# cvxgrp/pymde

Hardware: AMD Instinct MI355X
Metric: edges/sec/iter (avg_distortion fwd+bwd), n=1M |E|=50M d=2 (higher is better)
Workload: dtype f32; 1 GPU; BASELINE configs[3] / SURVEY 8d config 4a: n=1000000, |E|=50000000 uniform-random edges (out-degree 50), d=2, penalties.Log1p(1.5), weights in {1,2}; seeded on the device with torch.Generator(0) (the survey's recipe uses numpy default_rng(0): same distribution, another stream; --survey-seed builds that one); parallelism=single GPU, parameter_stream=codebook: 2 distinct weights ride in the packed half-edge word (4 B/half-edge)

## Files before the change

### include/mde_hip.h

```cpp
#ifndef MDE_HIP_H_
#define MDE_HIP_H_

#include <stdint.h>

#ifdef __cplusplus
extern "C" {
#endif

#define MDE_ABI_VERSION 2

#define MDE_OK 0
#define MDE_E_INVALID (-1)
#define MDE_E_SELF_EDGE (-2)
#define MDE_E_RANGE (-3)
#define MDE_E_TOO_LARGE (-4)
#define MDE_E_HIP (-5)
#define MDE_E_UNSUPPORTED (-6)

const char* mde_last_error(void);
int mde_abi_version(void);

enum {
  MDE_F_NONE = 0,
  MDE_F_LINEAR = 1,
// ... 21 lines not shown
  MDE_F_L_LOGISTIC = 39,
  MDE_F_L_FRACTIONAL = 40,
  MDE_F_L_SOFT_FRACTIONAL = 41,
  MDE_F_L_CLIPPED_QUADRATIC = 42,
  MDE_F_L_LOG1P = 43
};

typedef struct mde_func {
  int32_t kind;
  int32_t kind_neg;
  const float* a0;
  const float* a1;
  int32_t a0_scalar;
  int32_t a1_scalar;
  float s0, s1, s2;
  float n0, n1, n2;
  int32_t layout;
  const float* e0;
  const float* e1;
} mde_func;

typedef struct mde_plan mde_plan;

int mde_plan_create(int64_t n, int64_t p, const int64_t* edges, int64_t row_lo, int64_t row_hi,
                    void* stream, mde_plan** out);
int mde_plan_destroy(mde_plan* plan);
int64_t mde_plan_n(const mde_plan* plan);
int64_t mde_plan_p(const mde_plan* plan);
int64_t mde_plan_half_edges(const mde_plan* plan);
int64_t mde_plan_row_lo(const mde_plan* plan);
int64_t mde_plan_row_hi(const mde_plan* plan);
const int32_t* mde_plan_rowptr(const mde_plan* plan);
const int32_t* mde_plan_nbr(const mde_plan* plan);
const int32_t* mde_plan_eid(const mde_plan* plan);

int mde_plan_export(const mde_plan* plan, int32_t* rowptr_out, int32_t* nbr_out, int32_t* eid_out,
                    void* stream);

int mde_shard_bounds(int64_t n, int64_t p, const int64_t* edges, int32_t world,
                     int64_t* bounds_host, void* stream);

int mde_plan_expand(const mde_plan* plan, const float* in_edge, float* out_half, void* stream);

int mde_plan_layout(mde_plan* plan, int32_t d, void* stream);
int mde_plan_function_hint(mde_plan* plan, int32_t kind, int32_t kind_neg);
int64_t mde_plan_layout_half_edges(const mde_plan* plan, int32_t layout);
int mde_plan_expand_codebook(const mde_plan* plan, const float* in_edge, float* out_half,
                             int32_t* n_values_host, void* stream);
int mde_plan_expand_bytes(const mde_plan* plan, const float* in_edge, float* out_half,
                          int32_t* n_values_host, void* stream);
int mde_plan_expand_layout(const mde_plan* plan, int32_t layout, const float* in_edge,
                           float* out_half, void* stream);
int mde_plan_ring_info(const mde_plan* plan, int64_t* info_host);
int mde_plan_row_order(mde_plan* plan, int32_t mode, void* stream, double* info_host);
int mde_plan_loss_double(const mde_plan* plan, double* dst, void* stream);

int mde_edges_deduplicate(int64_t n, int64_t p, const int64_t* edges, int64_t* edges_out,
                          int64_t* count_host, void* stream);
int mde_edges_count_unique(int64_t n, int64_t p, const int64_t* edges, int64_t* edges_out,
                           float* weights_out, int64_t* count_host, void* stream);
int mde_knn(int64_t n, int32_t nf, const float* data, int32_t k, int32_t* idx_out, float* d2_out,
            float* sqn_work, void* stream);
int mde_row_sqnorm(int64_t n, int32_t nf, const float* data, float* out, void* stream);
int mde_ann_search(int32_t nf, int32_t k, int32_t flags, int64_t n_q, const float* Q, const float* q_sqn,
                   int64_t n_qpos, const int32_t* q_map, int64_t n_b, const float* B, const float* b_sqn,
                   int64_t n_bpos, const int32_t* b_map, int64_t n_lists, const int64_t* offsets,
                   int32_t n_probe, const int32_t* probe, int64_t n_tiles, const int64_t* tiles,
                   int32_t* idx_out, float* d2_out, void* stream);
int mde_ann_centroids(int64_t n, int32_t nf, const float* data, int64_t n_members, const int32_t* members,
                      int64_t n_lists, const int64_t* offsets, float* centroids, void* stream);
int mde_sparse_validate(int64_t n, int32_t nf, int64_t nnz, const int64_t* indptr, const int32_t* indices,
                        const float* values, void* stream);
int mde_sparse_knn(int64_t n, int32_t nf, int64_t nnz, const int64_t* indptr, const int32_t* indices,
                   const float* values, int32_t k, int32_t* idx_out, float* d2_out, float* sqn_work,
                   void* stream);
int mde_sparse_distances(int64_t n, int32_t nf, int64_t nnz, const int64_t* indptr, const int32_t* indices,
                         const float* values, int64_t p, const int64_t* edges, float* out, void* stream);
int mde_graph_shortest_paths(const mde_plan* plan, const float* w, float max_length,
                             double retain_fraction, uint64_t seed, int64_t capacity,
                             int64_t* edges_out, float* dist_out, int64_t* count_host, void* stream);
int mde_knn_pairs(int64_t n, int32_t k, const int32_t* idx, const float* val, float max_value,
                  int64_t* pairs_out, void* stream);
int mde_graph_knn(const mde_plan* plan, const float* w, float max_length, int32_t direct, int32_t k,
                  int32_t* idx_out, float* dist_out, void* stream);
int mde_sample_edges(int64_t n, int64_t num_edges, uint64_t seed, const int64_t* exclude,
                     int64_t n_exclude, int64_t* edges_out, int64_t* count_host, void* stream);

int mde_average_distortion(mde_plan* plan, const float* X, int32_t d, const mde_func* f,
                           float grad_scale, float* grad, float* loss_out, void* stream);

int mde_differences(int64_t n, int64_t p, const int64_t* edges, const float* X, int32_t d,
                    float* diff_out , void* stream);
int mde_distances(int64_t n, int64_t p, const int64_t* edges, const float* X, int32_t d,
                  float* dist_out , void* stream);
int mde_distances_backward(const mde_plan* plan, const float* X, int32_t d, const float* gout,
                           float* grad , void* stream);
int mde_distortions(int64_t p, const float* dist, const mde_func* f, float* out, float* dout,
                    void* stream);

int mde_scatter(const mde_plan* plan, const float* X, int32_t d, const float* gnorm,
                const float* dist, float scale, float* grad, void* stream);

int mde_center(int64_t n, int32_t d, float* Z, double* work, void* stream);
int mde_anchor_rows(int64_t n_anchors, int32_t d, const int64_t* anchors, const float* values,
                    float* Z, void* stream);
int mde_sphere_rows(int64_t n, int32_t d, const float* X, float* Z, float radius, void* stream);
// ... 83 lines not shown
```

### pymde_amd/_lib.py

```python
import ctypes
import os
import threading

import torch

_HERE = os.path.dirname(os.path.abspath(__file__))
LIB_PATH = os.path.join(_HERE, "libmde_hip.so")

c_i32, c_i64, c_f32 = ctypes.c_int32, ctypes.c_int64, ctypes.c_float
c_vp = ctypes.c_void_p

MDE_OK = 0
MDE_E_INVALID, MDE_E_SELF_EDGE, MDE_E_RANGE = -1, -2, -3
MDE_E_TOO_LARGE, MDE_E_HIP, MDE_E_UNSUPPORTED = -4, -5, -6


class MdeFunc(ctypes.Structure):
    _fields_ = [("kind", c_i32), ("kind_neg", c_i32), ("a0", c_vp), ("a1", c_vp),
                ("a0_scalar", c_i32), ("a1_scalar", c_i32),
                ("s0", c_f32), ("s1", c_f32), ("s2", c_f32),
                ("n0", c_f32), ("n1", c_f32), ("n2", c_f32), ("layout", c_i32),
                ("e0", c_vp), ("e1", c_vp)]


class MdeTurnDesc(ctypes.Structure):
    _fields_ = [("plan", c_vp), ("func", c_vp), ("n", c_i64), ("d", c_i32), ("kind", c_i32),
                ("X", c_vp * 2), ("g", c_vp), ("g_prev", c_vp), ("dir", c_vp), ("loss_dev", c_vp),
                ("board", c_vp), ("work", c_vp), ("status", c_vp), ("lbfgs", c_vp),
                ("host_dst", c_vp), ("tail_src", c_vp), ("read_bytes", c_i64),
                ("host_loss", c_vp), ("host_status", c_vp), ("host_board", c_vp), ("seq", ctypes.c_double),
                ("pre_id", ctypes.c_double)]


SYMBOLS = {
    "mde_last_error": (ctypes.c_char_p, []),
    "mde_abi_version": (c_i32, []),
    "mde_plan_create": (c_i32, [c_i64, c_i64, c_vp, c_i64, c_i64, c_vp, ctypes.POINTER(c_vp)]),
    "mde_plan_destroy": (c_i32, [c_vp]),
    "mde_plan_n": (c_i64, [c_vp]),
    "mde_plan_p": (c_i64, [c_vp]),
    "mde_plan_half_edges": (c_i64, [c_vp]),
    "mde_plan_row_lo": (c_i64, [c_vp]),
    "mde_plan_row_hi": (c_i64, [c_vp]),
    "mde_plan_rowptr": (c_vp, [c_vp]),
    "mde_plan_nbr": (c_vp, [c_vp]),
    "mde_plan_eid": (c_vp, [c_vp]),
    "mde_plan_export": (c_i32, [c_vp, c_vp, c_vp, c_vp, c_vp]),
    "mde_shard_bounds": (c_i32, [c_i64, c_i64, c_vp, c_i32, ctypes.POINTER(c_i64), c_vp]),
    "mde_plan_expand": (c_i32, [c_vp, c_vp, c_vp, c_vp]),
    "mde_plan_layout": (c_i32, [c_vp, c_i32, c_vp]),
    "mde_plan_layout_half_edges": (c_i64, [c_vp, c_i32]),
    "mde_plan_ring_info": (c_i32, [c_vp, ctypes.POINTER(c_i64)]),
    "mde_plan_row_order": (c_i32, [c_vp, c_i32, c_vp, ctypes.POINTER(ctypes.c_double)]),
    "mde_plan_function_hint": (c_i32, [c_vp, c_i32, c_i32]),
    "mde_plan_loss_double": (c_i32, [c_vp, c_vp, c_vp]),
    "mde_center_step_begin": (c_i32, [c_i64, c_i32, c_vp, c_vp, c_f32, c_vp, c_vp, c_vp]),
    "mde_center_step_end": (c_i32, [c_i64, c_i32, c_vp, c_vp, ctypes.c_double, c_vp]),
    "mde_lbfgs_dev_stage": (c_i32, [c_vp, c_vp, c_vp, c_vp, c_f32, c_vp, c_vp]),
    "mde_lbfgs_dev_finish": (c_i32, [c_vp, c_vp, c_vp, c_vp, c_vp, c_vp]),
    "mde_lbfgs_dev_dots": (c_i32, [c_vp]),
    "mde_rank_reduce": (c_i32, [c_i32, c_i32, ctypes.c_uint64, c_vp, c_vp, c_i32, c_vp, c_vp]),
    "mde_plan_expand_codebook": (c_i32, [c_vp, c_vp, c_vp, ctypes.POINTER(c_i32), c_vp]),
    "mde_plan_expand_bytes": (c_i32, [c_vp, c_vp, c_vp, ctypes.POINTER(c_i32), c_vp]),
    "mde_plan_expand_layout": (c_i32, [c_vp, c_i32, c_vp, c_vp, c_vp]),
    "mde_edges_deduplicate": (c_i32, [c_i64, c_i64, c_vp, c_vp, ctypes.POINTER(c_i64), c_vp]),
    "mde_edges_count_unique": (c_i32, [c_i64, c_i64, c_vp, c_vp, c_vp, ctypes.POINTER(c_i64), c_vp]),
    "mde_knn": (c_i32, [c_i64, c_i32, c_vp, c_i32, c_vp, c_vp, c_vp, c_vp]),
    "mde_row_sqnorm": (c_i32, [c_i64, c_i32, c_vp, c_vp, c_vp]),
    "mde_ann_search": (c_i32, [c_i32, c_i32, c_i32, c_i64, c_vp, c_vp, c_i64, c_vp, c_i64, c_vp, c_vp, c_i64, c_vp,
                               c_i64, c_vp, c_i32, c_vp, c_i64, c_vp, c_vp, c_vp, c_vp]),
    "mde_ann_centroids": (c_i32, [c_i64, c_i32, c_vp, c_i64, c_vp, c_i64, c_vp, c_vp, c_vp]),
    "mde_knn_pairs": (c_i32, [c_i64, c_i32, c_vp, c_vp, c_f32, c_vp, c_vp]),
    "mde_sparse_validate": (c_i32, [c_i64, c_i32, c_i64, c_vp, c_vp, c_vp, c_vp]),
    "mde_sparse_knn": (c_i32, [c_i64, c_i32, c_i64, c_vp, c_vp, c_vp, c_i32, c_vp, c_vp, c_vp, c_vp]),
    "mde_sparse_distances": (c_i32, [c_i64, c_i32, c_i64, c_vp, c_vp, c_vp, c_i64, c_vp, c_vp, c_vp]),
    "mde_graph_knn": (c_i32, [c_vp, c_vp, c_f32, c_i32, c_i32, c_vp, c_vp, c_vp]),
    "mde_graph_shortest_paths": (c_i32, [c_vp, c_vp, c_f32, ctypes.c_double, ctypes.c_uint64, c_i64,
                                         c_vp, c_vp, ctypes.POINTER(c_i64), c_vp]),
    "mde_sample_edges": (c_i32, [c_i64, c_i64, ctypes.c_uint64, c_vp, c_i64, c_vp,
                                 ctypes.POINTER(c_i64), c_vp]),
    "mde_average_distortion": (c_i32, [c_vp, c_vp, c_i32, ctypes.POINTER(MdeFunc), c_f32, c_vp,
                                       c_vp, c_vp]),
    "mde_differences": (c_i32, [c_i64, c_i64, c_vp, c_vp, c_i32, c_vp, c_vp]),
    "mde_distances": (c_i32, [c_i64, c_i64, c_vp, c_vp, c_i32, c_vp, c_vp]),
    "mde_distances_backward": (c_i32, [c_vp, c_vp, c_i32, c_vp, c_vp, c_vp]),
    "mde_distortions": (c_i32, [c_i64, c_vp, ctypes.POINTER(MdeFunc), c_vp, c_vp, c_vp]),
    "mde_scatter": (c_i32, [c_vp, c_vp, c_i32, c_vp, c_vp, c_f32, c_vp, c_vp]),
    "mde_center": (c_i32, [c_i64, c_i32, c_vp, c_vp, c_vp]),
    "mde_anchor_rows": (c_i32, [c_i64, c_i32, c_vp, c_vp, c_vp, c_vp]),
    "mde_sphere_rows": (c_i32, [c_i64, c_i32, c_vp, c_vp, c_f32, c_vp]),
    "mde_std_tangent": (c_i32, [c_i64, c_i32, c_vp, c_vp, c_vp, c_vp]),
    "mde_std_retract": (c_i32, [c_i64, c_i32, c_vp, c_i32, c_vp, c_vp, c_vp]),
    "mde_center_step": (c_i32, [c_i64, c_i32, c_vp, c_vp, c_f32, c_vp, c_vp, c_vp]),
    "mde_std_retract_step": (c_i32, [c_i64, c_i32, c_vp, c_vp, c_f32, c_vp, c_i32, c_vp, c_vp, c_vp]),
    "mde_std_tangent_stats": (c_i32, [c_i64, c_i32, c_vp, c_vp, c_vp, c_vp, c_vp, c_vp]),
    "mde_gram": (c_i32, [c_i64, c_i32, c_i32, c_vp, c_vp, c_vp, c_vp, c_vp]),
    "mde_right_multiply": (c_i32, [c_i64, c_i32, c_i32, c_vp, c_vp, c_vp, c_vp]),
    "mde_right_multiply_add": (c_i32, [c_i64, c_i32, c_i32, c_vp, c_vp, c_f32, c_vp, c_vp, c_vp]),
    "mde_shift_rows": (c_i32, [c_i64, c_i32, c_vp, c_vp, c_vp]),
    "mde_row_scale": (c_i32, [c_i64, c_i32, c_vp, c_vp, c_vp]),
    "mde_weighted_degree": (c_i32, [c_vp, c_vp, c_vp, c_vp]),
    "mde_work_doubles": (c_i64, [c_i32]),
    "mde_axpy": (c_i32, [c_i64, c_f32, c_vp, c_vp, c_vp, c_vp]),
    "mde_vec_stats": (c_i32, [c_i64, c_vp, c_vp, c_vp, c_vp, c_vp, c_vp]),
    "mde_lbfgs_create": (c_i32, [c_i64, c_i32, ctypes.POINTER(c_vp)]),
# ... 79 lines not shown
```

### pymde_amd/average_distortion.py

```python
import ctypes

import torch

from pymde_amd import _lib
from pymde_amd import util


def _check_X(X, n=None, d=None):
    if not isinstance(X, torch.Tensor) or X.dim() != 2:
        raise ValueError("the embedding must be a 2-D tensor")
    if X.dtype != torch.float32:
        raise ValueError(
            "pymde_amd computes in float32; got an embedding of dtype %s (MDE.embed and "
            "MDE.average_distortion cast float64 inputs with a warning; the kernels themselves do not)" % X.dtype)
    util.require_cuda_device(X.device)
    if n is not None and X.shape[0] != n:
        raise ValueError("embedding has %d rows, the problem has %d items" % (X.shape[0], n))


class EdgePlan(object):

    def __init__(self, n_items, edges, row_lo=0, row_hi=None):
        lib = _lib.load()
        device = util.require_cuda_device(edges.device)
# ... 27 lines not shown
    @property
    def is_full(self):
        return self.row_lo == 0 and self.row_hi == self.n

    def expand(self, per_edge, layout=0):
        lib = _lib.load()
        t = per_edge.detach().to(device=self.device, dtype=torch.float32).contiguous().reshape(-1)
        if t.numel() != self.p:
            raise ValueError(
                "distortion function has %d parameters but the problem has %d edges"
                % (t.numel(), self.p))
        size = int(lib.mde_plan_layout_half_edges(self._handle, int(layout)))
        out = torch.empty(max(size, 1), dtype=torch.float32, device=self.device)
        with torch.cuda.device(self.device):
            _lib.check(lib.mde_plan_expand_layout(self._handle, int(layout), _lib.ptr(t),
                                                  _lib.ptr(out), _lib.stream_ptr(self.device)))
        return out

    def expand_codebook(self, per_edge):
        lib = _lib.load()
        t = per_edge.detach().to(device=self.device, dtype=torch.float32).contiguous().reshape(-1)
        if t.numel() != self.p:
            return None
        size = int(lib.mde_plan_layout_half_edges(self._handle, 1))
        out = torch.empty(max(size, 1), dtype=torch.float32, device=self.device)
        nv = ctypes.c_int32(0)
        with torch.cuda.device(self.device):
            _lib.check(lib.mde_plan_expand_codebook(self._handle, _lib.ptr(t), _lib.ptr(out),
                                                    ctypes.byref(nv), _lib.stream_ptr(self.device)))
        return out if nv.value > 0 else None

    def expand_bytes(self, per_edge):
        lib = _lib.load()
        t = per_edge.detach().to(device=self.device, dtype=torch.float32).contiguous().reshape(-1)
        if t.numel() != self.p:
            return None
        size = int(lib.mde_plan_layout_half_edges(self._handle, 1))
        out = torch.empty(max(size, 1), dtype=torch.float32, device=self.device)
        nv = ctypes.c_int32(0)
        with torch.cuda.device(self.device):
            _lib.check(lib.mde_plan_expand_bytes(self._handle, _lib.ptr(t), _lib.ptr(out),
                                                 ctypes.byref(nv), _lib.stream_ptr(self.device)))
        return out if nv.value > 0 else None

    def ring_info(self):
        lib = _lib.load()
        info = (ctypes.c_int64 * 16)()
        _lib.check(lib.mde_plan_ring_info(self._handle, info))
        names = ("built", "d", "rows_per_block", "row_blocks", "col_groups", "chunks", "ring_slots", "iterations",
                 "ring_half_edges", "padded_entries", "permuted", "hub_rows", "hub_half_edges", "hub_segments")
        out = {k: int(info[i]) for i, k in enumerate(names)}
        out["built"], out["permuted"] = bool(out["built"]), bool(out["permuted"])
        return out

    def row_order(self, mode=1):
        lib = _lib.load()
        info = (ctypes.c_double * 4)()
        with torch.cuda.device(self.device):
            _lib.check(lib.mde_plan_row_order(self._handle, int(mode), _lib.stream_ptr(self.device), info))
        return {"in_use": bool(info[0]), "mean_distance_before": float(info[1]),
                "mean_distance_after": float(info[2]), "levels": int(info[3])}

    def csr(self):
        lib = _lib.load()
        nloc = self.row_hi - self.row_lo
        rowptr = torch.empty(nloc + 1, dtype=torch.int32, device=self.device)
        nbr = torch.empty(max(self.half_edges, 1), dtype=torch.int32, device=self.device)
        eid = torch.empty(max(self.half_edges, 1), dtype=torch.int32, device=self.device)
        with torch.cuda.device(self.device):
            _lib.check(lib.mde_plan_export(self._handle, _lib.ptr(rowptr), _lib.ptr(nbr),
                                           _lib.ptr(eid), _lib.stream_ptr(self.device)))
        return rowptr, nbr[:self.half_edges], eid[:self.half_edges]

    def __del__(self):
        h = getattr(self, "_handle", None)
        if h is not None and h.value:
            try:
                _lib.load().mde_plan_destroy(h)
            except Exception:
                pass
            self._handle = None


class Binding(object):

    def __init__(self, plan, function):
        self.plan = plan
        self.function = function
        self.spec = function._hip_spec() if hasattr(function, "_hip_spec") else None
        self._struct = None
        self._keep = None
        self._key = None
        self.codebook = False
        self.byte_stream = False
        self.stream_kind = None

    @property
    def fused(self):
        return self.spec is not None

    def _param_key(self, spec):
        return tuple((a.data_ptr(), a._version, a.numel(), str(a.device)) for a in spec.arrays()) + (
            spec.kind, spec.kind_neg, spec.scalars, spec.scalars_neg)

    def struct(self, d):
        lib = _lib.load()
# ... 186 lines not shown
```

### pymde_amd/csrc/mde_ring.hip

```cpp
#include <algorithm>
#include <chrono>
#include <cmath>
#include <cstring>
#include <vector>

#include "mde_ring.h"

#ifndef MDE_RING_BUCKETS
#define MDE_RING_BUCKETS 32
#endif
__global__ __launch_bounds__(64) void k_ring_assign(int nloc, int R, int Q, int NC, int C, int contiguous,
                                                    const int32_t* __restrict__ rowptr,
                                                    const int32_t* __restrict__ nbr, uint32_t* __restrict__ wmap,
                                                    int32_t* __restrict__ wrows) {
  constexpr int B = MDE_RING_BUCKETS, NCWP = MDE_RING_NCW <= 8 ? 8 : 16, LPW = 64 / NCWP, BPL = B / LPW;
  static_assert(MDE_RING_NCW <= 16 && B % LPW == 0 && B <= 64, "lane map of k_ring_assign");
  __shared__ int hist[B];
  __shared__ float cpre[B];
  const int wg = blockIdx.x, rb = wg / Q, g = wg % Q, lane = threadIdx.x;
  const int j_lo = (int)(((int64_t)g * NC + Q - 1) / Q), j_hi = (int)(((int64_t)(g + 1) * NC + Q - 1) / Q);
  const int nj = max(1, j_hi - j_lo);
  const int r0 = rb * R, nr = min(R, nloc - r0);
  const int w = lane / LPW, bg = lane % LPW;
  uint32_t* out = wmap + (size_t)wg * R;
// ... 343 lines not shown
    caps[i] = 0;
    return;
  }
  const int nrows_w = max(1, wrows[i]);
  const int per_it = nrows_w < 64 ? nrows_w : 64;
  const int walk = 2 * ((NC / Q + SPAN + 1) / (SPAN + 1));
  const int need = max((seg[i + 1] - seg[i] + per_it - 1) / per_it, walk);
  caps[i] = (factor * need + 64 + 4 + 3) & ~3;
}

__device__ __forceinline__ int ring_place_wave(bool act, int rc, int lane) {
  const unsigned long long lt = (1ull << lane) - 1ull;
  int rank = 0, par = 0, oddacc = 0;
  for (int c = 0; c < 32; ++c) {
    const unsigned long long m = __ballot(act && rc == c);
    if (rc == c) {
      rank = __popcll(m & lt);
      par = oddacc & 1;
    }
    oddacc += __popcll(m) & 1;
  }
  const int half = (rank + par) & 1;
  int quarter = 0;
  for (int h = 0; h < 2; ++h) {
    int oa = 0;
    for (int c = 0; c < 16; ++c) {
      const unsigned long long m = __ballot(act && half == h && (rc & 15) == c);
      if (half == h && (rc & 15) == c) quarter = (__popcll(m & lt) + (oa & 1)) & 1;
      oa += __popcll(m) & 1;
    }
  }
  int pos = 0;
  for (int g = 0; g < 4; ++g) {
    const unsigned long long m = __ballot(act && half * 2 + quarter == g);
    if (half * 2 + quarter == g) pos = __popcll(m & lt);
  }
  return half * 32 + quarter * 16 + pos;
}

__global__ __launch_bounds__(MDE_BLOCK) void k_ring_pack(int64_t nit, int nseg, const int32_t* __restrict__ iter_base,
                                                         const int32_t* __restrict__ src_base,
                                                         const int32_t* __restrict__ it_ent,
                                                         const int32_t* __restrict__ it_cnt,
                                                         const int32_t* __restrict__ it_m,
                                                         const uint32_t* __restrict__ keys,
                                                         const uint32_t* __restrict__ vals,
                                                         const int32_t* __restrict__ hrow,
                                                         const int32_t* __restrict__ nbr,
                                                         const int32_t* __restrict__ eid, int R, int Q, int C, int S,
                                                         int ring_off, int JB, int d, int row_lo, int place, int count_all,
                                                         uint32_t* __restrict__ packed,
                                                         int32_t* __restrict__ peid, uint32_t* __restrict__ hdr) {
  __shared__ uint8_t s_taken[MDE_BLOCK / 64][64], s_free[MDE_BLOCK / 64][64];
  const int lane = threadIdx.x & 63, wv = threadIdx.x >> 6;
  const int64_t nw = ((int64_t)gridDim.x * MDE_BLOCK) >> 6;
  const uint32_t JM = (1u << JB) - 1u;
  const int sh = ring_cls_shift(d), cm = ring_cls_mask(d);
  const uint32_t cbytes = (uint32_t)C * 4u * (uint32_t)d;
  for (int64_t itb = (int64_t)blockIdx.x * (MDE_BLOCK / 64); itb < nit; itb += nw) {
    const int64_t it = itb + wv;
    const bool valid = it < nit;
    int64_t src = it;
    if (valid && src_base) {
      int lo = 0, hi = nseg;
      while (hi - lo > 1) {
        const int mid = (lo + hi) >> 1;
        if ((int64_t)iter_base[mid] <= it) lo = mid; else hi = mid;
      }
      src = (int64_t)src_base[lo] + (it - (int64_t)iter_base[lo]);
    }
    const int cw = valid ? __builtin_amdgcn_readfirstlane(it_cnt[src]) : 0;
    const int cnt = cw & 0xff;
    const bool act = valid && lane < cnt;
    uint32_t key = 0, q = 0, col = 0, rowaddr = 0, ring = 0;
    int grow = 0, rcls = 0;
    if (act) {
      const int pos = it_ent[(size_t)src * 64 + lane];
      key = keys[pos];
      q = vals[pos];
      const int rb = (int)((key >> JB) / MDE_RING_NCW) / Q;
      grow = hrow[q];
      rowaddr = (uint32_t)(grow - rb * R) * 4u * (uint32_t)d;
      const uint32_t j = key & JM;
      col = (uint32_t)nbr[q];
      ring = (uint32_t)ring_off + (j % (uint32_t)S) * cbytes + (col - j * (uint32_t)C) * 4u * (uint32_t)d;
      rcls = (int)((rowaddr >> sh) & (uint32_t)cm);
    }
    s_taken[wv][lane] = 0;
    __syncthreads();
    int l = lane;
    if (place) l = ring_place_wave(act, rcls, lane);
    if (act) s_taken[wv][l] = 1;
    __syncthreads();
    {
      const bool fr = !s_taken[wv][lane];
      const unsigned long long fm = __ballot(fr);
      if (fr) s_free[wv][__popcll(fm & ((1ull << lane) - 1ull))] = (uint8_t)lane;
    }
    __syncthreads();
    const bool counts = act && (count_all || (uint32_t)(row_lo + grow) < col);
    const int ncount = __popcll(__ballot(counts));
    const uint32_t lclass = ncount == 0 ? 0u : (ncount == cnt ? 1u : 2u);
    const uint32_t m = valid ? (uint32_t)__builtin_amdgcn_readfirstlane(it_m[src]) : 0u;
    const uint32_t need = max((uint32_t)(cw >> 8), m);
    const uint32_t mpad = valid ? (uint32_t)__builtin_amdgcn_readfirstlane(it_m[src & ~(int64_t)1]) : 0u;
    const size_t base = ((size_t)(it >> 2) * 64) * 4 + (size_t)(it & 3);
    if (act) {
      packed[base + (size_t)l * 4] = ring_pack_word(d, rowaddr, ring);
      peid[base + (size_t)l * 4] = eid[q];
    } else if (valid) {
      const int lf = s_free[wv][lane - cnt];
      packed[base + (size_t)lf * 4] = ring_pack_word(d, (uint32_t)(R + (lf & 31)) * 4u * (uint32_t)d,
                                                     (uint32_t)ring_off + (mpad % (uint32_t)S) * cbytes);
      peid[base + (size_t)lf * 4] = -1;
    }
    if (lane == 0 && valid) {
      hdr[MDE_RING_HW * it] = m;
      hdr[MDE_RING_HW * it + 1] = need;
      hdr[MDE_RING_HW * it + 2] = lclass;
      hdr[MDE_RING_HW * it + 3] = (cnt < 64 ? MDE_RING_H3_PAD : 0u) | ((uint32_t)cnt << 8);
    }
    __syncthreads();
  }
}

__global__ __launch_bounds__(MDE_BLOCK) void k_ring_block_class(int64_t nblocks, uint32_t* __restrict__ hdr) {
  const int64_t b = (int64_t)blockIdx.x * MDE_BLOCK + threadIdx.x;
  if (b >= nblocks) return;
  bool any0 = false, any1 = false, any2 = false;
  for (int q = 0; q < 4; ++q) {
    const uint32_t* h = hdr + (size_t)MDE_RING_HW * (4 * b + q);
    if ((h[3] >> 8) == 0u) continue;
    any0 |= h[2] == 0u;
    any1 |= h[2] == 1u;
    any2 |= h[2] == 2u;
  }
  const uint32_t cls = (any2 || (any0 && any1)) ? 2u : (any1 ? 1u : 0u);
  hdr[(size_t)MDE_RING_HW * 4 * b + 3] = (hdr[(size_t)MDE_RING_HW * 4 * b + 3] & ~3u) | cls;
  for (int t = 0; t < 2; ++t) {
    uint32_t* h0 = hdr + (size_t)MDE_RING_HW * (4 * b + 2 * t);
    uint32_t* h1 = h0 + MDE_RING_HW;
    uint32_t need = h0[0];
    if ((h0[3] >> 8) != 0u) need = max(need, h0[1]);
    if ((h1[3] >> 8) != 0u) need = max(need, h1[1]);
    h0[1] = need;
  }
}

__global__ __launch_bounds__(MDE_BLOCK) void k_ring_stats(int64_t nit, const uint32_t* __restrict__ hdr,
                                                          unsigned long long* __restrict__ stats) {
  unsigned long long a = 0, b = 0, c = 0;
  for (int64_t i = (int64_t)blockIdx.x * MDE_BLOCK + threadIdx.x; i < nit; i += (int64_t)gridDim.x * MDE_BLOCK) {
    a += (hdr[MDE_RING_HW * i + 3] & MDE_RING_H3_PAD) ? 1u : 0u;
    b += hdr[MDE_RING_HW * i + 2] == 1u;
    c += hdr[MDE_RING_HW * i + 2] == 2u;
  }
  a = mde_wave_sum(a);
  b = mde_wave_sum(b);
  c = mde_wave_sum(c);
  if ((threadIdx.x & 63) == 0) {
    atomicAdd(&stats[0], a);
    atomicAdd(&stats[1], b);
    atomicAdd(&stats[2], c);
  }
// ... 982 lines not shown
    memcpy(&fv, &vals[i], sizeof(float));
    if (!std::isfinite(fv) || std::fabs(fv) > 1.0e6f) ok = false;
  }
  if (!ok) {
    (void)hipFree(dtable);
    return MDE_OK;
  }
  std::sort(vals.begin(), vals.end());
  const int nv = (int)vals.size();
  std::vector<unsigned int> tb(MDE_RING_BX_VALUES, 0u);
  for (int i = 0; i < nv; ++i) tb[1 + i] = vals[i];
  unsigned int* table = reinterpret_cast<unsigned int*>(out_half) + L.H / 4;
  err = hipMemcpyAsync(table, tb.data(), MDE_RING_BX_VALUES * sizeof(unsigned int), hipMemcpyHostToDevice, st);
  if (err == hipSuccess) {
    hipLaunchKernelGGL(k_bytes_pack, dim3(mde_grid(L.H, MDE_BLOCK, 4096)), dim3(MDE_BLOCK), 0, st, L.H, L.eid, in_edge, table, nv,
                       reinterpret_cast<uint8_t*>(out_half));
    err = hipGetLastError();
  }
  if (err == hipSuccess) err = hipStreamSynchronize(st);
  (void)hipFree(dtable);
  if (err != hipSuccess) return mde_hip_fail(err, "byte-index stream: pack", __FILE__, __LINE__);
  *n_values_host = nv;
  return MDE_OK;
}

extern "C" int mde_plan_loss_double(const mde_plan* plan, double* dst, void* stream) {
  if (!plan || !dst) return MDE_E_INVALID;
  MDE_HIP(hipMemcpyAsync(dst, plan->partials + MDE_PARTIALS_LOSS_D, sizeof(double), hipMemcpyDeviceToDevice, mde_stream(stream)));
  return MDE_OK;
}

extern "C" int mde_plan_ring_info(const mde_plan* plan, int64_t* info) {
  if (!plan || !info) return MDE_E_INVALID;
  const mde_ring_layout& L = plan->ring;
  for (int i = 0; i < 16; ++i) info[i] = 0;
  if (!L.packed) return MDE_OK;
  info[0] = 1;
  info[1] = L.d;
  info[2] = L.rows_per_block;
  info[3] = L.n_row_blocks;
  info[4] = L.col_groups;
  info[5] = L.n_chunks;
  info[6] = L.slots;
  info[7] = L.n_iters;
  info[8] = plan->H - L.hub_half_edges;
  info[9] = L.H;
  info[10] = L.slot_row ? 1 : 0;
  info[11] = L.n_hub_rows;
  info[12] = L.hub_half_edges;
  info[13] = L.n_hub_segs;
  return MDE_OK;
}

extern "C" int mde_plan_expand_layout(const mde_plan* plan, int32_t layout, const float* in_edge,
                                      float* out_half, void* stream) {
  if (!plan || !in_edge || !out_half) return MDE_E_INVALID;
  if (layout == 0) return mde_plan_expand(plan, in_edge, out_half, stream);
  if (layout != 1 || !plan->ring.eid) {
    mde_set_error("mde_plan_expand_layout: the LDS-ring layout has not been built");
    return MDE_E_INVALID;
  }
  if (plan->ring.H == 0) return MDE_OK;
  hipLaunchKernelGGL(k_expand_ring, dim3(mde_grid(plan->ring.H, MDE_BLOCK, 4096)), dim3(MDE_BLOCK), 0,
                     mde_stream(stream), plan->ring.H, plan->ring.eid, in_edge, out_half);
  MDE_LAUNCH_CHECK();
  return MDE_OK;
}

template <int D>
__global__ __launch_bounds__(MDE_BLOCK) void k_hub_rows(const int32_t* __restrict__ hub_rows, const int32_t* __restrict__ hub_seg,
                                                        int row_lo, const int32_t* __restrict__ nbr,
                                                        const int32_t* __restrict__ eid, const float* __restrict__ e0,
                                                        const float* __restrict__ e1, int e0_scalar, int e1_scalar,
                                                        const float* __restrict__ X, FnRuntime fn, float inv_p, int count_all,
                                                        double* __restrict__ partial) {
  __shared__ double smem[8];
  const int sgi = blockIdx.x;
  const int hi = hub_seg[4 * sgi], beg = hub_seg[4 * sgi + 1], end = hub_seg[4 * sgi + 2];
  const int64_t v = (int64_t)row_lo + hub_rows[hi];
  float xv[D];
#pragma unroll
  for (int c = 0; c < D; ++c) xv[c] = X[v * D + c];
  const float e0s = e0_scalar ? e0[0] : 0.0f;
  const float e1s = (e1 && e1_scalar) ? e1[0] : 0.0f;
  double acc[D], loss = 0.0;
#pragma unroll
  for (int c = 0; c < D; ++c) acc[c] = 0.0;
  for (int h = beg + (int)threadIdx.x; h < end; h += MDE_BLOCK) {
    const int u = nbr[h], k = eid[h];
    const float p0 = e0_scalar ? e0s : e0[k];
    const float p1 = (e1 && !e1_scalar) ? e1[k] : e1s;
    float diff[D], ss = 0.0f;
#pragma unroll
    for (int c = 0; c < D; ++c) {
      diff[c] = xv[c] - X[(size_t)u * D + c];
      ss = fmaf(diff[c], diff[c], ss);
    }
    float f, gd;
    fn.eval(ss, p0, p1, f, gd);
    const float g = mde_fix_g(gd * inv_p);
    if (count_all || v < (int64_t)u) loss += (double)f;
#pragma unroll
    for (int c = 0; c < D; ++c) acc[c] += (double)(g * diff[c]);
  }
#pragma unroll
  for (int c = 0; c < D; ++c) {
// ... 113 lines not shown
```

### pymde_amd/csrc/mde_ring_kernel.h

```cpp
#pragma once
#include <algorithm>
#include <cstring>
#include <type_traits>
#include <vector>

#include "mde_ring.h"
#define COMMA ,

#define MDE_RING23(FN, LIN)                                    \
  do {                                                         \
    FN fn{a};                                                  \
    int rc;                                                    \
    if (A.d == 2)                                              \
      rc = launch_ring<2, FN, LIN>(A, fn, nblocks);            \
    else                                                       \
      rc = launch_ring<3, FN, LIN>(A, fn, nblocks);            \
    return rc == MDE_OK ? 1 : rc;                              \
  } while (0)

typedef uint32_t ring_u4 __attribute__((ext_vector_type(4)));
typedef float ring_f4 __attribute__((ext_vector_type(4)));

template <int D>
struct RingVec;
// ... 488 lines not shown
          ready = __builtin_amdgcn_readfirstlane(fl_pre);
#endif
          if (__builtin_expect(need >= ready, 0)) {
#if MDE_RING_ABLATE
            const unsigned long long tp0 = RING_CLK();
#endif
            for (;;) {
#if MDE_RING_FWORDS
              {
                ring_i4 fv;
                asm volatile("ds_read_b128 %0, %1\n\ts_waitcnt lgkmcnt(0)" : "=&v"(fv) : "v"(f_addr) : "memory");
                ready = __builtin_amdgcn_readfirstlane(min4(fv));
              }
#else
              ready = __builtin_amdgcn_readfirstlane(ring_ctrl_load(f_addr));
#endif
#if MDE_RING_ABLATE
              ++cs_trips;
              if (cs_trips > MDE_RING_SPINMAX) {
                if (lane == 0) {
                  const int k = atomicAdd(&g_ring_ndiag, 1);
                  if (k < 64) {
                    int* r = g_ring_diag[k];
                    r[0] = 1; r[1] = blockIdx.x; r[2] = wave; r[3] = need; r[4] = ready; r[5] = 0; r[6] = u * 4 + q; r[7] = NB;
                  }
                }
                cs_trips = 0;
                ready = need + 1;
                break;
              }
#endif
              if (need < ready) break;
              __builtin_amdgcn_s_sleep(MDE_RING_CSLEEP);
            }
#if MDE_RING_ABLATE
            cs_poll += RING_CLK() - tp0;
#endif
          }
          asm volatile("" ::: "memory");
        }
      };
#if MDE_RING_FWORDS
      auto prefetch_landed = [&]() __attribute__((always_inline)) { fl_pre = *(lds_cvint4)(L + CTRL_F); };
#else
      auto prefetch_landed = [&]() __attribute__((always_inline)) { fl_pre = *(lds_cvint)(L + CTRL_F); };
#endif
      const uint32_t rel_addr[2] = {lane == 0 ? 4u * (uint32_t)wave : 128u + 4u * (uint32_t)(lane & 31),
                                    lane == 8 ? 4u * (uint32_t)wave : 128u + 4u * (uint32_t)(lane & 31)};
      auto release_to = [&](int u, int q) __attribute__((always_inline)) {
        ring_ctrl_store_counted(L, CTRL_PROG + rel_addr[q >> 1], (int)hv[u]);
      };

      Pre xa, xb;
      float acc[D];
      auto block_body = [&](auto lc_tag, int u, int b) __attribute__((always_inline)) {
#pragma unroll
        for (int h = 0; h < 2; ++h) {
          const int q = 2 * h;
          const int un = h == 0 ? u : (u + 1) % PFB, qn = (q + 2) & 3;
          wait_pair(un, qn);
          const Pre xna = issue_x(pq[un][qn], (a0_scalar || PS != 0) ? a0s : wq[un][qn], bx4(bq[un], qn));
          const Pre xnb = issue_x(pq[un][qn + 1], (a0_scalar || PS != 0) ? a0s : wq[un][qn + 1], bx4(bq[un], qn + 1));
          release_to((u + 1) % PFB, q);
          prefetch_landed();
          const float p1a = a1_arr ? a1[((size_t)((ib >> 2) + b) * 64 + lane) * 4 + q] : a1s;
          const float p1b = a1_arr ? a1[((size_t)((ib >> 2) + b) * 64 + lane) * 4 + q + 1] : a1s;
          const bool lc2 = decltype(lc_tag)::value == 2;
          const uint32_t hma = lc2 ? (uint32_t)__builtin_amdgcn_readlane((int)hv[u], 4 * q) : 0u;
          const uint32_t hmb = lc2 ? (uint32_t)__builtin_amdgcn_readlane((int)hv[u], 4 * q + 4) : 0u;
          finish(lc_tag, pq[u][q], xa, acc, p1a, hma);
          if (HAS_GRAD) ring_ld<D>(L + GR_OFF + row_of(pq[u][q + 1]), acc);
          finish(lc_tag, pq[u][q + 1], xb, acc, p1b, hmb);
          if (HAS_GRAD) ring_ld<D>(L + GR_OFF + row_of(pq[un][qn]), acc);
          xa = xna;
          xb = xnb;
        }
      };
#pragma unroll
      for (int u = 0; u < PFB; ++u) load_block(u, u);
      release_to(0, 0);
      wait_pair(0, 0);
      xa = issue_x(pq[0][0], (a0_scalar || PS != 0) ? a0s : wq[0][0], bx4(bq[0], 0));
      xb = issue_x(pq[0][1], (a0_scalar || PS != 0) ? a0s : wq[0][1], bx4(bq[0], 1));
      release_to(0, 2);
      prefetch_landed();
      if (HAS_GRAD) ring_ld<D>(L + GR_OFF + row_of(pq[0][0]), acc);
      for (int base = 0; base < NB; base += PFB) {
#pragma unroll
        for (int u = 0; u < PFB; ++u) {
          const int b = base + u;
          if (b < NB) {
            const int bcls = __builtin_amdgcn_readlane((int)hv[u], 3) & 3;
            if (bcls == 0)
              block_body(std::integral_constant<int, 0>(), u, b);
            else if (bcls == 1)
              block_body(std::integral_constant<int, 1>(), u, b);
            else
              block_body(std::integral_constant<int, 2>(), u, b);
          }
          load_block(u, b + PFB);
        }
      }
#if MDE_RING_ABLATE
      if ((dbg & 512) && lane == 0 && blockIdx.x < 1024) {
        atomicAdd(&g_ring_probe[0][blockIdx.x], RING_CLK() - cs_t0);
        atomicAdd(&g_ring_probe[1][blockIdx.x], cs_poll);
        atomicAdd(&g_ring_probe[2][blockIdx.x], cs_trips);
      }
#endif
    }
    if constexpr (Fn::kRingFused) loss = fmaf(loss, 0.6931471805599453f, loss2) * (1.0f / Fn::kParamScale);
    ring_ctrl_store_counted(L, CTRL_PROG + 4u * (uint32_t)wave, MDE_RING_DONE);
    __builtin_amdgcn_s_waitcnt(0x0F70);
  }
  __syncthreads();
  if (HAS_GRAD && slot_row) {
    const int32_t* sr = slot_row + (size_t)rb * R;
    if (fold) {
      unsigned int* sync = reinterpret_cast<unsigned int*>(partial + (size_t)Q * nloc * D) + 2 * rb;
      int* tk = reinterpret_cast<int*>(L + 512);
      if (tid == 0) *tk = (int)__hip_atomic_fetch_add(&sync[0], 1u, __ATOMIC_RELAXED, __HIP_MEMORY_SCOPE_AGENT);
      __syncthreads();
      const bool second = *tk != 0;
      float* mine = partial + (size_t)qg * nloc * D;
      const float* other = partial + (size_t)(1 - qg) * nloc * D;
      if (!second) {
        for (int sl = tid; sl < R; sl += BS) {
          const int r = sr[sl];
          if (r < 0) continue;
#pragma unroll
          for (int c = 0; c < D; ++c)
            __hip_atomic_store(mine + (size_t)r * D + c, GR[sl * D + c], __ATOMIC_RELAXED, __HIP_MEMORY_SCOPE_AGENT);
        }
        __builtin_amdgcn_s_waitcnt(0x0F70);
        __syncthreads();
        if (tid == 0) __hip_atomic_store(&sync[1], 1u, __ATOMIC_RELAXED, __HIP_MEMORY_SCOPE_AGENT);
      } else {
        if (tid == 0) {
          while (__hip_atomic_load(&sync[1], __ATOMIC_RELAXED, __HIP_MEMORY_SCOPE_AGENT) == 0u) __builtin_amdgcn_s_sleep(2);
          __hip_atomic_store(&sync[1], 0u, __ATOMIC_RELAXED, __HIP_MEMORY_SCOPE_AGENT);
          __hip_atomic_store(&sync[0], 0u, __ATOMIC_RELAXED, __HIP_MEMORY_SCOPE_AGENT);
        }
        __syncthreads();
        for (int sl = tid; sl < R; sl += BS) {
          const int r = sr[sl];
          if (r < 0) continue;
#pragma unroll
          for (int c = 0; c < D; ++c) {
            const float o = __hip_atomic_load(other + (size_t)r * D + c, __ATOMIC_RELAXED, __HIP_MEMORY_SCOPE_AGENT);
            const float m = GR[sl * D + c];
            grad[(size_t)(row_lo + r) * D + c] = (qg == 0 ? m + o : o + m) * grad_scale;
          }
        }
      }
      __syncthreads();
    } else {
      float* dst = (Q == 1) ? grad + (size_t)row_lo * D : partial + (size_t)qg * nloc * D;
      const float sc = (Q == 1) ? grad_scale : 1.0f;
      for (int sl = tid; sl < R; sl += BS) {
        const int r = sr[sl];
        if (r < 0) continue;
#pragma unroll
        for (int c = 0; c < D; ++c) dst[(size_t)r * D + c] = GR[sl * D + c] * sc;
      }
    }
  } else if (HAS_GRAD && fold) {
    unsigned int* sync = reinterpret_cast<unsigned int*>(partial + (size_t)Q * nloc * D) + 2 * rb;
    int* tk = reinterpret_cast<int*>(L + 512);
    if (tid == 0) *tk = (int)__hip_atomic_fetch_add(&sync[0], 1u, __ATOMIC_RELAXED, __HIP_MEMORY_SCOPE_AGENT);
    __syncthreads();
    const bool second = *tk != 0;
    float* mine = partial + ((size_t)qg * nloc + r0) * D;
    const float* other = partial + ((size_t)(1 - qg) * nloc + r0) * D;
    float* grow = grad + (size_t)(row_lo + r0) * D;
    if (!second) {
      if constexpr (D == 2) {
        for (int i = tid; i < nr; i += BS)
          __hip_atomic_store(reinterpret_cast<double*>(mine) + i, reinterpret_cast<const double*>(GR)[i], __ATOMIC_RELAXED,
                             __HIP_MEMORY_SCOPE_AGENT);
      } else {
        for (int i = tid; i < nr * D; i += BS) __hip_atomic_store(mine + i, GR[i], __ATOMIC_RELAXED, __HIP_MEMORY_SCOPE_AGENT);
      }
      __builtin_amdgcn_s_waitcnt(0x0F70);
      __syncthreads();
      if (tid == 0) __hip_atomic_store(&sync[1], 1u, __ATOMIC_RELAXED, __HIP_MEMORY_SCOPE_AGENT);
    } else {
      if (tid == 0) {
        while (__hip_atomic_load(&sync[1], __ATOMIC_RELAXED, __HIP_MEMORY_SCOPE_AGENT) == 0u) __builtin_amdgcn_s_sleep(2);
        __hip_atomic_store(&sync[1], 0u, __ATOMIC_RELAXED, __HIP_MEMORY_SCOPE_AGENT);
        __hip_atomic_store(&sync[0], 0u, __ATOMIC_RELAXED, __HIP_MEMORY_SCOPE_AGENT);
      }
      __syncthreads();
      if constexpr (D == 2) {
        for (int i = tid; i < nr; i += BS) {
          const double o = __hip_atomic_load(reinterpret_cast<const double*>(other) + i, __ATOMIC_RELAXED, __HIP_MEMORY_SCOPE_AGENT);
          const float2 ov = *reinterpret_cast<const float2*>(&o);
          const float2 mv = reinterpret_cast<const float2*>(GR)[i];
          float2 r;
          r.x = (qg == 0 ? mv.x + ov.x : ov.x + mv.x) * grad_scale;
          r.y = (qg == 0 ? mv.y + ov.y : ov.y + mv.y) * grad_scale;
          reinterpret_cast<float2*>(grow)[i] = r;
        }
      } else {
        for (int i = tid; i < nr * D; i += BS) {
          const float o = __hip_atomic_load(other + i, __ATOMIC_RELAXED, __HIP_MEMORY_SCOPE_AGENT);
          grow[i] = (qg == 0 ? GR[i] + o : o + GR[i]) * grad_scale;
        }
      }
    }
    __syncthreads();
  } else if (HAS_GRAD) {
    float* grow = (Q == 1) ? grad + (size_t)(row_lo + r0) * D : partial + ((size_t)qg * nloc + r0) * D;
    const float sc = (Q == 1) ? grad_scale : 1.0f;
    for (int i = tid; i < nr * D; i += BS) grow[i] = GR[i] * sc;
  }
  double* red = reinterpret_cast<double*>(L);
  unsigned int* ticket = reinterpret_cast<unsigned int*>(loss_partials + MDE_MAX_PARTIALS);
  const double v = mde_wave_sum((double)loss);
  if (lane == 0) red[wave] = v;
  __syncthreads();
  if (tid == 0) {
    double s = 0.0;
    for (int i = 0; i < NCW; ++i) s += red[i];
    mde_st_partial(loss_partials + blockIdx.x, s);
  }
  int* last_flag = reinterpret_cast<int*>(L + 256);
  __builtin_amdgcn_s_waitcnt(0x0F70);
  __syncthreads();
  if (tid == 0) {
    const unsigned int k = __hip_atomic_fetch_add(ticket, 1u, __ATOMIC_RELAXED, __HIP_MEMORY_SCOPE_AGENT);
    *last_flag = (k == gridDim.x - 1u) ? 1 : 0;
    if (*last_flag) __hip_atomic_store(ticket, 0u, __ATOMIC_RELAXED, __HIP_MEMORY_SCOPE_AGENT);
  }
  __syncthreads();
  if (!*last_flag) return;
  double t = 0.0;
  for (int i = tid; i < (int)gridDim.x; i += BS) t += mde_ld_partial(loss_partials + i);
  t = mde_wave_sum(t);
  __syncthreads();
  if (lane == 0) red[wave] = t;
  __syncthreads();
  if (tid == 0) {
    double s = 0.0;
    for (int i = 0; i < BS / 64; ++i) s += red[i];
    *loss_out = (float)(s * loss_scale);
    loss_partials[MDE_PARTIALS_LOSS_D] = s * loss_scale;
  }
}

template <class V>
__global__ __launch_bounds__(MDE_BLOCK) void k_ring_combine(int64_t m, int Q, const V* __restrict__ partial,
                                                            float scale, V* __restrict__ out) {
  constexpr int W = sizeof(V) / sizeof(float);
  const int64_t i = (int64_t)blockIdx.x * MDE_BLOCK + threadIdx.x;
  if (i >= m) return;
  V a[8];
#pragma unroll
  for (int q = 0; q < 8; ++q)
    if (q < Q) a[q] = partial[(size_t)q * m + i];
  float s[W];
#pragma unroll
  for (int k = 0; k < W; ++k) s[k] = reinterpret_cast<const float*>(&a[0])[k];
#pragma unroll
  for (int q = 1; q < 8; ++q)
    if (q < Q) {
#pragma unroll
      for (int k = 0; k < W; ++k) s[k] += reinterpret_cast<const float*>(&a[q])[k];
// ... 132 lines not shown
```

Measured before the change: 312.6 billion edges/s/iter.

## Pin paired-iteration rows to same lanes, split gradient accumulators, vectorize fold stores

Ring layout placement now pins a row from odd iterations to the lane that row held in the preceding even iteration, so consecutive half-edges in a lane share a row. The kernel keeps a second accumulator for the second half-edge of each pair, which breaks the serial read-modify-write dependency on one accumulator. The cross-block gradient fold and the write-back use 16-byte vector stores and loads, with the loads batched eight per thread to raise memory-level parallelism. A diagnostic kernel that counts pair sharing is also added. The changes add register pressure and make the layout placement more complex.

```diff
diff --git a/include/mde_hip.h b/include/mde_hip.h
--- a/include/mde_hip.h
+++ b/include/mde_hip.h
@@ -97,6 +97,7 @@
 int mde_plan_expand_layout(const mde_plan* plan, int32_t layout, const float* in_edge,
                            float* out_half, void* stream);
 int mde_plan_ring_info(const mde_plan* plan, int64_t* info_host);
+int mde_plan_ring_check(const mde_plan* plan, int64_t* out_host, void* stream);
 int mde_plan_row_order(mde_plan* plan, int32_t mode, void* stream, double* info_host);
 int mde_plan_loss_double(const mde_plan* plan, double* dst, void* stream);
 
diff --git a/pymde_amd/_lib.py b/pymde_amd/_lib.py
--- a/pymde_amd/_lib.py
+++ b/pymde_amd/_lib.py
@@ -51,6 +51,7 @@
     "mde_plan_layout": (c_i32, [c_vp, c_i32, c_vp]),
     "mde_plan_layout_half_edges": (c_i64, [c_vp, c_i32]),
     "mde_plan_ring_info": (c_i32, [c_vp, ctypes.POINTER(c_i64)]),
+    "mde_plan_ring_check": (c_i32, [c_vp, ctypes.POINTER(c_i64), c_vp]),
     "mde_plan_row_order": (c_i32, [c_vp, c_i32, c_vp, ctypes.POINTER(ctypes.c_double)]),
     "mde_plan_function_hint": (c_i32, [c_vp, c_i32, c_i32]),
     "mde_plan_loss_double": (c_i32, [c_vp, c_vp, c_vp]),
diff --git a/pymde_amd/average_distortion.py b/pymde_amd/average_distortion.py
--- a/pymde_amd/average_distortion.py
+++ b/pymde_amd/average_distortion.py
@@ -103,6 +103,13 @@
         out = {k: int(info[i]) for i, k in enumerate(names)}
         out["built"], out["permuted"] = bool(out["built"]), bool(out["permuted"])
         return out
+
+    def ring_check(self):
+        lib = _lib.load()
+        out = (ctypes.c_int64 * 3)()
+        with torch.cuda.device(self.device):
+            _lib.check(lib.mde_plan_ring_check(self._handle, out, _lib.stream_ptr(self.device)))
+        return {"split": int(out[0]), "shared": int(out[1]), "pairs": int(out[2])}
 
     def row_order(self, mode=1):
         lib = _lib.load()
diff --git a/pymde_amd/csrc/mde_ring.hip b/pymde_amd/csrc/mde_ring.hip
--- a/pymde_amd/csrc/mde_ring.hip
+++ b/pymde_amd/csrc/mde_ring.hip
@@ -419,6 +419,7 @@
                                                          uint32_t* __restrict__ packed,
                                                          int32_t* __restrict__ peid, uint32_t* __restrict__ hdr) {
   __shared__ uint8_t s_taken[MDE_BLOCK / 64][64], s_free[MDE_BLOCK / 64][64];
+  __shared__ uint32_t s_prow[MDE_BLOCK / 64][64];
   const int lane = threadIdx.x & 63, wv = threadIdx.x >> 6;
   const int64_t nw = ((int64_t)gridDim.x * MDE_BLOCK) >> 6;
   const uint32_t JM = (1u << JB) - 1u;
@@ -454,10 +455,34 @@
       rcls = (int)((rowaddr >> sh) & (uint32_t)cm);
     }
     s_taken[wv][lane] = 0;
+    s_prow[wv][lane] = 0xffffffffu;
     __syncthreads();
+    const bool second = (it & 1) != 0;
     int l = lane;
-    if (place) l = ring_place_wave(act, rcls, lane);
-    if (act) s_taken[wv][l] = 1;
+    if (!second) {
+      if (place) l = ring_place_wave(act, rcls, lane);
+      if (act) {
+        s_taken[wv][l] = 1;
+        s_prow[wv][l] = rowaddr;
+      }
+    }
+    __syncthreads();
+    int pin = -1;
+    if (second) {
+      const uint32_t prow = s_prow[wv - 1][lane];
+#pragma unroll 8
+      for (int k = 0; k < 64; ++k)
+        if ((uint32_t)__builtin_amdgcn_readlane((int)prow, k) == rowaddr) pin = k;
+      pin = act ? pin : -1;
+      if (place) l = ring_place_wave(act && pin < 0, rcls, lane);
+      if (pin >= 0) {
+        l = pin;
+        s_taken[wv][l] = 1;
+      }
+    }
+    __syncthreads();
+    const bool moved = second && act && pin < 0 && s_taken[wv][l];
+    if (second && act && !moved) s_taken[wv][l] = 1;
     __syncthreads();
     {
       const bool fr = !s_taken[wv][lane];
@@ -465,6 +490,9 @@
       if (fr) s_free[wv][__popcll(fm & ((1ull << lane) - 1ull))] = (uint8_t)lane;
     }
     __syncthreads();
+    const unsigned long long mvm = __ballot(moved);
+    const int nmoved = __popcll(mvm);
+    if (moved) l = s_free[wv][__popcll(mvm & ((1ull << lane) - 1ull))];
     const bool counts = act && (count_all || (uint32_t)(row_lo + grow) < col);
     const int ncount = __popcll(__ballot(counts));
     const uint32_t lclass = ncount == 0 ? 0u : (ncount == cnt ? 1u : 2u);
@@ -476,7 +504,7 @@
       packed[base + (size_t)l * 4] = ring_pack_word(d, rowaddr, ring);
       peid[base + (size_t)l * 4] = eid[q];
     } else if (valid) {
-      const int lf = s_free[wv][lane - cnt];
+      const int lf = s_free[wv][nmoved + lane - cnt];
       packed[base + (size_t)lf * 4] = ring_pack_word(d, (uint32_t)(R + (lf & 31)) * 4u * (uint32_t)d,
                                                      (uint32_t)ring_off + (mpad % (uint32_t)S) * cbytes);
       peid[base + (size_t)lf * 4] = -1;
@@ -1565,6 +1593,57 @@
   return MDE_OK;
 }
 
+__global__ __launch_bounds__(MDE_BLOCK) void k_ring_pair_check(int64_t npairs, const uint32_t* __restrict__ packed, int d, int R,
+                                                               unsigned long long* __restrict__ out) {
+  const int lane = threadIdx.x & 63;
+  const int64_t nw = ((int64_t)gridDim.x * MDE_BLOCK) >> 6;
+  const uint32_t mask = d == 2 ? 0xfff8u : 0xfffcu, dummy = (uint32_t)R * 4u * (uint32_t)d;
+  unsigned long long split = 0, shared = 0, pairs = 0;
+  for (int64_t pr = ((int64_t)blockIdx.x * MDE_BLOCK + threadIdx.x) >> 6; pr < npairs; pr += nw) {
+    const int64_t it = 2 * pr;
+    const size_t base = ((size_t)(it >> 2) * 64 + (size_t)lane) * 4 + (size_t)(it & 3);
+    const uint32_t ra = packed[base] & mask, rb = packed[base + 1] & mask;
+    int found = -1;
+    for (int k = 0; k < 64; ++k)
+      if ((uint32_t)__builtin_amdgcn_readlane((int)ra, k) == rb) found = k;
+    const bool real = rb < dummy;
+    split += __popcll(__ballot(real && found >= 0 && found != lane));
+    shared += __popcll(__ballot(real && found >= 0));
+    ++pairs;
+  }
+  if (lane == 0) {
+    atomicAdd(&out[0], split);
+    atomicAdd(&out[1], shared);
+    atomicAdd(&out[2], pairs);
+  }
+}
+
+extern "C" int mde_plan_ring_check(const mde_plan* plan, int64_t* out_host, void* stream) {
+  if (!plan || !out_host) return MDE_E_INVALID;
+  const mde_ring_layout& L = plan->ring;
+  for (int i = 0; i < 3; ++i) out_host[i] = 0;
+  if (!L.packed || L.n_iters == 0) return MDE_OK;
+  hipStream_t st = mde_stream(stream);
+  unsigned long long* dout = nullptr;
+  hipError_t e = hipMalloc(&dout, 3 * sizeof(unsigned long long));
+  if (e == hipSuccess) e = hipMemsetAsync(dout, 0, 3 * sizeof(unsigned long long), st);
+  if (e == hipSuccess) {
+    hipLaunchKernelGGL(k_ring_pair_check, dim3(mde_grid(L.n_iters / 2 * 64, MDE_BLOCK, 4096)), dim3(MDE_BLOCK), 0, st,
+                       L.n_iters / 2, L.packed, L.d, L.rows_per_block, dout);
+    e = hipGetLastError();
+  }
+  unsigned long long h[3] = {0, 0, 0};
+  if (e == hipSuccess) e = hipMemcpyAsync(h, dout, sizeof(h), hipMemcpyDeviceToHost, st);
+  if (e == hipSuccess) e = hipStreamSynchronize(st);
+  if (dout) (void)hipFree(dout);
+  if (e != hipSuccess) {
+    mde_set_error("mde_plan_ring_check: %s", hipGetErrorString(e));
+    return MDE_E_HIP;
+  }
+  for (int i = 0; i < 3; ++i) out_host[i] = (int64_t)h[i];
+  return MDE_OK;
+}
+
 extern "C" int mde_plan_expand_layout(const mde_plan* plan, int32_t layout, const float* in_edge,
                                       float* out_half, void* stream) {
   if (!plan || !in_edge || !out_half) return MDE_E_INVALID;
diff --git a/pymde_amd/csrc/mde_ring_kernel.h b/pymde_amd/csrc/mde_ring_kernel.h
--- a/pymde_amd/csrc/mde_ring_kernel.h
+++ b/pymde_amd/csrc/mde_ring_kernel.h
@@ -564,7 +564,7 @@
       };
 
       Pre xa, xb;
-      float acc[D];
+      float acc[D], accb[D];
       auto block_body = [&](auto lc_tag, int u, int b) __attribute__((always_inline)) {
 #pragma unroll
         for (int h = 0; h < 2; ++h) {
@@ -581,9 +581,16 @@
           const uint32_t hma = lc2 ? (uint32_t)__builtin_amdgcn_readlane((int)hv[u], 4 * q) : 0u;
           const uint32_t hmb = lc2 ? (uint32_t)__builtin_amdgcn_readlane((int)hv[u], 4 * q + 4) : 0u;
           finish(lc_tag, pq[u][q], xa, acc, p1a, hma);
-          if (HAS_GRAD) ring_ld<D>(L + GR_OFF + row_of(pq[u][q + 1]), acc);
-          finish(lc_tag, pq[u][q + 1], xb, acc, p1b, hmb);
-          if (HAS_GRAD) ring_ld<D>(L + GR_OFF + row_of(pq[un][qn]), acc);
+          if (HAS_GRAD) {
+            const bool same = row_of(pq[u][q + 1]) == row_of(pq[u][q]);
+#pragma unroll
+            for (int c = 0; c < D; ++c) accb[c] = same ? acc[c] : accb[c];
+          }
+          finish(lc_tag, pq[u][q + 1], xb, accb, p1b, hmb);
+          if (HAS_GRAD) {
+            ring_ld<D>(L + GR_OFF + row_of(pq[un][qn]), acc);
+            ring_ld<D>(L + GR_OFF + row_of(pq[un][qn + 1]), accb);
+          }
           xa = xna;
           xb = xnb;
         }
@@ -596,7 +603,10 @@
       xb = issue_x(pq[0][1], (a0_scalar || PS != 0) ? a0s : wq[0][1], bx4(bq[0], 1));
       release_to(0, 2);
       prefetch_landed();
-      if (HAS_GRAD) ring_ld<D>(L + GR_OFF + row_of(pq[0][0]), acc);
+      if (HAS_GRAD) {
+        ring_ld<D>(L + GR_OFF + row_of(pq[0][0]), acc);
+        ring_ld<D>(L + GR_OFF + row_of(pq[0][1]), accb);
+      }
       for (int base = 0; base < NB; base += PFB) {
 #pragma unroll
         for (int u = 0; u < PFB; ++u) {
@@ -654,14 +664,25 @@
           __hip_atomic_store(&sync[0], 0u, __ATOMIC_RELAXED, __HIP_MEMORY_SCOPE_AGENT);
         }
         __syncthreads();
-        for (int sl = tid; sl < R; sl += BS) {
-          const int r = sr[sl];
-          if (r < 0) continue;
-#pragma unroll
-          for (int c = 0; c < D; ++c) {
-            const float o = __hip_atomic_load(other + (size_t)r * D + c, __ATOMIC_RELAXED, __HIP_MEMORY_SCOPE_AGENT);
-            const float m = GR[sl * D + c];
-            grad[(size_t)(row_lo + r) * D + c] = (qg == 0 ? m + o : o + m) * grad_scale;
+        for (int s0 = 0; s0 < R; s0 += 8 * BS) {
+          int rr[8];
+          float o[8][D];
+#pragma unroll
+          for (int k = 0; k < 8; ++k) rr[k] = s0 + tid + k * BS < R ? sr[s0 + tid + k * BS] : -1;
+#pragma unroll
+          for (int k = 0; k < 8; ++k)
+#pragma unroll
+            for (int c = 0; c < D; ++c)
+              o[k][c] = __hip_atomic_load(other + (size_t)max(rr[k], 0) * D + c, __ATOMIC_RELAXED, __HIP_MEMORY_SCOPE_AGENT);
+#pragma unroll
+          for (int k = 0; k < 8; ++k) {
+            if (rr[k] < 0) continue;
+            const int sl = s0 + tid + k * BS;
+#pragma unroll
+            for (int c = 0; c < D; ++c) {
+              const float m = GR[sl * D + c];
+              grad[(size_t)(row_lo + rr[k]) * D + c] = (qg == 0 ? m + o[k][c] : o[k][c] + m) * grad_scale;
+            }
           }
         }
       }
@@ -685,14 +706,16 @@
     float* mine = partial + ((size_t)qg * nloc + r0) * D;
     const float* other = partial + ((size_t)(1 - qg) * nloc + r0) * D;
     float* grow = grad + (size_t)(row_lo + r0) * D;
+    static_assert(GR_OFF % 16 == 0, "16-byte accumulator pieces");
+    const bool vec = ((reinterpret_cast<uintptr_t>(mine) | reinterpret_cast<uintptr_t>(other) | reinterpret_cast<uintptr_t>(grow)) & 15) == 0;
+    const int n4 = vec ? (nr * D) >> 2 : 0, n1 = nr * D;
+    const ring_f4* GR4 = reinterpret_cast<const ring_f4*>(GR);
     if (!second) {
-      if constexpr (D == 2) {
-        for (int i = tid; i < nr; i += BS)
-          __hip_atomic_store(reinterpret_cast<double*>(mine) + i, reinterpret_cast<const double*>(GR)[i], __ATOMIC_RELAXED,
-                             __HIP_MEMORY_SCOPE_AGENT);
-      } else {
-        for (int i = tid; i < nr * D; i += BS) __hip_atomic_store(mine + i, GR[i], __ATOMIC_RELAXED, __HIP_MEMORY_SCOPE_AGENT);
-      }
+      for (int i = tid; i < n4; i += BS) {
+        const ring_f4 v4 = GR4[i];
+        asm volatile("global_store_dwordx4 %0, %1, off sc1" ::"v"(reinterpret_cast<ring_f4*>(mine) + i), "v"(v4) : "memory");
+      }
+      for (int i = (n4 << 2) + tid; i < n1; i += BS) __hip_atomic_store(mine + i, GR[i], __ATOMIC_RELAXED, __HIP_MEMORY_SCOPE_AGENT);
       __builtin_amdgcn_s_waitcnt(0x0F70);
       __syncthreads();
       if (tid == 0) __hip_atomic_store(&sync[1], 1u, __ATOMIC_RELAXED, __HIP_MEMORY_SCOPE_AGENT);
@@ -703,20 +726,30 @@
         __hip_atomic_store(&sync[0], 0u, __ATOMIC_RELAXED, __HIP_MEMORY_SCOPE_AGENT);
       }
       __syncthreads();
-      if constexpr (D == 2) {
-        for (int i = tid; i < nr; i += BS) {
-          const double o = __hip_atomic_load(reinterpret_cast<const double*>(other) + i, __ATOMIC_RELAXED, __HIP_MEMORY_SCOPE_AGENT);
-          const float2 ov = *reinterpret_cast<const float2*>(&o);
-          const float2 mv = reinterpret_cast<const float2*>(GR)[i];
-          float2 r;
-          r.x = (qg == 0 ? mv.x + ov.x : ov.x + mv.x) * grad_scale;
-          r.y = (qg == 0 ? mv.y + ov.y : ov.y + mv.y) * grad_scale;
-          reinterpret_cast<float2*>(grow)[i] = r;
-        }
-      } else {
-        for (int i = tid; i < nr * D; i += BS) {
-          const float o = __hip_atomic_load(other + i, __ATOMIC_RELAXED, __HIP_MEMORY_SCOPE_AGENT);
-          grow[i] = (qg == 0 ? GR[i] + o : o + GR[i]) * grad_scale;
+      const ring_f4* o4p = reinterpret_cast<const ring_f4*>(other);
+      for (int i0 = 0; i0 < n4; i0 += 8 * BS) {
+        ring_f4 o[8];
+#pragma unroll
+        for (int k = 0; k < 8; ++k)
+          asm volatile("global_load_dwordx4 %0, %1, off sc1" : "=v"(o[k]) : "v"(o4p + min(i0 + tid + k * BS, n4 - 1)) : "memory");
+        asm volatile("s_waitcnt vmcnt(0)" : "+v"(o[0]), "+v"(o[1]), "+v"(o[2]), "+v"(o[3]), "+v"(o[4]), "+v"(o[5]), "+v"(o[6]), "+v"(o[7])::"memory");
+#pragma unroll
+        for (int k = 0; k < 8; ++k) {
+          const int i = i0 + tid + k * BS;
+          if (i < n4) {
+            const ring_f4 m = GR4[i];
+            reinterpret_cast<ring_f4*>(grow)[i] = (qg == 0 ? m + o[k] : o[k] + m) * grad_scale;
+          }
+        }
+      }
+      for (int i0 = n4 << 2; i0 < n1; i0 += 8 * BS) {
+        float o[8];
+#pragma unroll
+        for (int k = 0; k < 8; ++k) o[k] = __hip_atomic_load(other + min(i0 + tid + k * BS, n1 - 1), __ATOMIC_RELAXED, __HIP_MEMORY_SCOPE_AGENT);
+#pragma unroll
+        for (int k = 0; k < 8; ++k) {
+          const int i = i0 + tid + k * BS;
+          if (i < n1) grow[i] = (qg == 0 ? GR[i] + o[k] : o[k] + GR[i]) * grad_scale;
         }
       }
     }
@@ -724,7 +757,9 @@
   } else if (HAS_GRAD) {
     float* grow = (Q == 1) ? grad + (size_t)(row_lo + r0) * D : partial + ((size_t)qg * nloc + r0) * D;
     const float sc = (Q == 1) ? grad_scale : 1.0f;
-    for (int i = tid; i < nr * D; i += BS) grow[i] = GR[i] * sc;
+    const int n4 = (reinterpret_cast<uintptr_t>(grow) & 15) == 0 ? (nr * D) >> 2 : 0;
+    for (int i = tid; i < n4; i += BS) reinterpret_cast<ring_f4*>(grow)[i] = reinterpret_cast<const ring_f4*>(GR)[i] * sc;
+    for (int i = (n4 << 2) + tid; i < nr * D; i += BS) grow[i] = GR[i] * sc;
   }
   double* red = reinterpret_cast<double*>(L);
   unsigned int* ticket = reinterpret_cast<unsigned int*>(loss_partials + MDE_MAX_PARTIALS);
```

After: 319.8 billion edges/s/iter (median of 6 runs). +2.3%, better.
